# Cobalt-27/CompactFusion

Measured on AMD Instinct MI355X. Metric: residual_compressed_activation_exchange_throughput, higher is better.
Workload: dtype f16

## Files before the change

### compactfusion_amd/csrc/cfx_absmean.hip

```cpp
#include <hip/hip_runtime.h>
#include <hip/hip_ext.h>
#include <stdint.h>
#include <stdio.h>
#include <stdlib.h>
#include <string.h>
#include <algorithm>
#include "cfx.h"
#include "cfx_internal.h"
#include "cfx_device.h"
#include "cfx_host.h"

#define CFX_I_FLAG_LR_FACTORS_ONLY 0x100
#define CFX_I_FLAG_LR_ABS 0x200
extern "C" CFX_HIDDEN size_t cfx_i_lr_workspace_bytes_any(int N, int C, int rank, int batch);
extern "C" CFX_HIDDEN void cfx_i_lr_factor_offsets(int N, int C, int rank, size_t* offU16, size_t* offV16, size_t* per);

template <bool EMIT_BITS, int US, bool WT = false, int NW = WAVES, bool PUB = false, bool KEEP = false, bool TAG = false>
__device__ __forceinline__ void absmean_stats_body(const cfx_comp_item& it, int N, int C, int R, int CB, int bx, int by,
                                                   u64* rowpart, u64 (*sm)[TILE_C], Probe probe = Probe(),
                                                   h16x8* xk = nullptr, h16x8* bk = nullptr, TagArena ta = TagArena()) {
#define SSTAMP(k) probe.at(k)
    const TileCoord t = tile_coord_at(bx, by, N, C, R);
    const int cb = bx;
    u64* colpart = rowpart + (size_t)N * CB;
// ... 263 lines not shown
            for (int k = 0; k < 8; ++k) u[k] = (k0 + k < K) ? U[(size_t)r * K + k0 + k] : (h16)0;
#pragma unroll
            for (int e = 0; e < 8; ++e)
#pragma unroll
                for (int k = 0; k < 8; ++k) acc[j][e] += (float)(h16)(u[k] * v[e][k]);
        }
    }
#pragma unroll
    for (int j = 0; j < RPT; ++j) {
        const int r = t.r0 + t.w + j * WAVES;
        if (r >= t.r1) continue;
        h16x8 bv = (h16x8)(h16)0, xv = (h16x8)(h16)0;
        if (base) bv = ld8(base + (size_t)r * C + t.c);
        unsigned byte;
        if (QUANT) {
            xv = ld8(x + (size_t)r * C + t.c);
            const h16x8 d = xv - bv;
            byte = 0;
#pragma unroll
            for (int i = 0; i < 8; ++i) byte |= (d[i] >= (h16)0 ? 1u : 0u) << i;
            pk[(size_t)r * C8 + (t.c >> 3)] = (unsigned char)byte;
        } else byte = pk[(size_t)r * C8 + (t.c >> 3)];
        if (!upd) continue;
        h16x8 o;
#pragma unroll
        for (int e = 0; e < 8; ++e) {
            const h16 sc = (h16)acc[j][e];
            const h16 recv = ((byte >> e) & 1u) ? sc : -sc;
            o[e] = base ? (h16)(bv[e] + recv) : recv;
        }
        if (QUANT && !ef) o = xv;
        st8(out + (size_t)r * C + t.c, o);
    }
}

#ifndef WATCH_SLEEP
#define WATCH_SLEEP 4
#endif
#ifndef INT2_FLAG_SLEEP
#define INT2_FLAG_SLEEP 2
#endif
__device__ __forceinline__ void scales_watch(const TagArena& ta, int N, int C, int c0, int r0, long long timeout) {
    const int tid = threadIdx.x;
    if (tid < 2) {
        const u64* w = tid ? ta.tU + min(r0, N - 1) : ta.tV + min(c0 + ((r0 >> 1) & (TILE_C - 1)), C - 1);
        SpinClock clk;
        while (!tag_is(ld_wt(w), ta.tagbits)) {
            __builtin_amdgcn_s_sleep(WATCH_SLEEP);
            if (clk.expired(timeout)) break;
        }
    }
    lds_barrier();
}
template <int ROWS, bool WATCH = true>
__device__ __forceinline__ bool scales_from_tagged(const TagArena& ta, int N, int C, int c0, int r0, u16* s16, long long timeout, unsigned* err) {
    static_assert(ROWS <= TILE_C, "one token word per thread (512 threads = the column block's channels)");
    const int tid = threadIdx.x;
    const u64* pv = ta.tV + min(c0 + tid, C - 1);
    const u64* pu = ta.tU + min(r0 + tid, N - 1);
    SpinClock clk;
    if (WATCH) scales_watch(ta, N, C, c0, r0, timeout);
    for (;;) {
        const u64 v = ld_wt(pv);
        const u64 u = tid < ROWS ? ld_wt(pu) : ta.tagbits;
        const bool ok = tag_is(v, ta.tagbits) && tag_is(u, ta.tagbits);
        s16[tid] = (u16)v;
        if (tid < ROWS) s16[TILE_C + tid] = (u16)u;
        if (!__syncthreads_or(ok ? 0 : 1)) return true;
        __builtin_amdgcn_s_sleep(2);
        if (__syncthreads_or(!ok && clk.expired(timeout) ? 1 : 0)) {
            if (tid == 0) gate_fail(err);
            return false;
        }
    }
}

#ifndef ONEBIT_D_TAGGED
#define ONEBIT_D_TAGGED 0
#endif
template <int NW, int KR, int KL, bool ST>
__device__ __forceinline__ void binary_dequant_gated_body(const cfx_decomp_item& it, int N, int C, int R, int tile_x, int tile_y,
                                                         unsigned* gate, unsigned expect, unsigned* err, long long timeout, u32x4* lds,
                                                         Probe probe = Probe(), bool remote = false, bool tagged = false, TagArena ta = TagArena(),
                                                         u16* s16 = nullptr) {
    constexpr int K = KR + KL;
#define GSTAMP(k) do { if (ST && probe.on()) { asm volatile("s_waitcnt vmcnt(0)" ::: "memory"); probe.at(k); } } while (0)
    const TileCoord t = tile_coord_at(tile_x, tile_y, N, C, R);
    if (ST) { probe.at(0); probe.set(7, 4); }
    const unsigned char* pk = (const unsigned char*)it.packet;
    const int C8 = C >> 3;
    const u16* U = (const u16*)(pk + (size_t)N * C8);
    const u16* V = U + N;
    const h16* base = (const h16*)it.base;
    h16* out = (h16*)it.recon;
    const int cc = min(t.c, C - 8);
    h16x8 bv[KR];
    if (base) {
#pragma unroll
        for (int j = 0; j < KR; ++j) bv[j] = ld8nt(base + (size_t)min(t.r0 + t.w + NW * j, t.r1 - 1) * C + cc);
        if constexpr (KL > 0) {
            h16x8 tl[KL > 0 ? KL : 1];
#pragma unroll
            for (int j = 0; j < KL; ++j) tl[j] = ld8nt(base + (size_t)min(t.r0 + t.w + NW * (KR + j), t.r1 - 1) * C + cc);
#pragma unroll
            for (int j = 0; j < KL; ++j) lds[j * (NW * 64) + threadIdx.x] = __builtin_bit_cast(u32x4, tl[j]);
        }
    } else {
#pragma unroll
        for (int j = 0; j < KR; ++j) bv[j] = (h16x8)(h16)0;
    }
    GSTAMP(1);
    h16x8 v8;
    u16 ul;
    unsigned by[K];
    if (tagged) {
        scales_watch(ta, N, C, tile_x * TILE_C, t.r0, timeout);
        if (ST) probe.at(2);
#pragma unroll
        for (int j = 0; j < K; ++j) by[j] = ld_wt(pk + (size_t)min(t.r0 + t.w + NW * j, t.r1 - 1) * C8 + (cc >> 3));
        if (!scales_from_tagged<NW * K, false>(ta, N, C, tile_x * TILE_C, t.r0, s16, timeout, err)) return;
        v8 = __builtin_bit_cast(h16x8, *(const u16x8*)(s16 + 8 * t.lane));
        ul = s16[TILE_C + min(t.w + NW * min(t.lane, K - 1), t.r1 - 1 - t.r0)];
    } else if (!gate_wait<true>(gate, expect, err, timeout)) return;
    else if (remote) {
        if (ST) probe.at(2);
        u16x8 vb;
#pragma unroll
        for (int i = 0; i < 8; ++i) vb[i] = ld_sys(V + cc + i);
        v8 = __builtin_bit_cast(h16x8, vb);
        ul = ld_sys(U + min(t.r0 + t.w + NW * min(t.lane, K - 1), t.r1 - 1));
#pragma unroll
        for (int j = 0; j < K; ++j) by[j] = ld_sys(pk + (size_t)min(t.r0 + t.w + NW * j, t.r1 - 1) * C8 + (cc >> 3));
    } else {
        if (ST) probe.at(2);
        v8 = ld8_wt(V + cc);
        ul = ld_wt(U + min(t.r0 + t.w + NW * min(t.lane, K - 1), t.r1 - 1));
#pragma unroll
        for (int j = 0; j < K; ++j) by[j] = ld_wt(pk + (size_t)min(t.r0 + t.w + NW * j, t.r1 - 1) * C8 + (cc >> 3));
    }
    GSTAMP(3);
#pragma unroll
    for (int j = 0; j < K; ++j) {
        const int rr = t.r0 + t.w + NW * j;
        const h16 uj = hfrom((u16)__builtin_amdgcn_readlane((int)ul, j));
        if (rr < t.r1 && t.act) {
            const h16x8 s = v8 * uj;
            u16x8 sb = __builtin_bit_cast(u16x8, s);
#pragma unroll
            for (int i = 0; i < 8; ++i) sb[i] ^= ((by[j] >> i) & 1u) ? (u16)0 : (u16)0x8000;
            const h16x8 recv = __builtin_bit_cast(h16x8, sb);
            h16x8 bj = (h16x8)(h16)0;
            if (j < KR) bj = bv[j < KR ? j : 0];
            else if (base) bj = __builtin_bit_cast(h16x8, lds[(j - KR) * (NW * 64) + threadIdx.x]);
            st8nt(out + (size_t)rr * C + t.c, base ? (bj + recv) : recv);
        }
    }
    GSTAMP(4);
#undef GSTAMP
}

__device__ __forceinline__ void row_sums2_wt(const u64* rowpart, const unsigned* row32, int N, int CB, int m0, int m1, bool two, u64& s0, u64& s1) {
    s0 = 0; s1 = 0;
    for (int k0 = 0; k0 < CB; k0 += FUSED_RCH) {
        unsigned a[FUSED_RCH], b[FUSED_RCH];
#pragma unroll
        for (int j = 0; j < FUSED_RCH; ++j) a[j] = ld_wt(&row32[(size_t)min(k0 + j, CB - 1) * N + m0]);
        if (two) {
#pragma unroll
            for (int j = 0; j < FUSED_RCH; ++j) b[j] = ld_wt(&row32[(size_t)min(k0 + j, CB - 1) * N + m1]);
        } else {
#pragma unroll
            for (int j = 0; j < FUSED_RCH; ++j) b[j] = 0;
        }
        bool sat = false;
#pragma unroll
        for (int j = 0; j < FUSED_RCH; ++j) {
            s0 += (k0 + j < CB) ? a[j] : 0; s1 += (k0 + j < CB) ? b[j] : 0;
            sat |= (a[j] == PART_SAT) | (b[j] == PART_SAT);
        }
        if (sat) {
            for (int j = 0; j < FUSED_RCH && k0 + j < CB; ++j) {
                if (a[j] == PART_SAT) s0 += ld_wt(&rowpart[(size_t)(k0 + j) * N + m0]) - (u64)PART_SAT;
                if (two && b[j] == PART_SAT) s1 += ld_wt(&rowpart[(size_t)(k0 + j) * N + m1]) - (u64)PART_SAT;
            }
        }
    }
}

template <bool GATED>
__device__ __forceinline__ void absmean_last_arriver_jobs(const cfx_comp_item& it, int N, int C, int CB, int P, int bx, u64* rowpart,
                                                          unsigned* tick, int per_byte, int eps_mode, u64 (*sm)[TILE_C], bool last_col,
                                                          bool last_all, Probe probe, unsigned* gate, unsigned gate_expect) {
    constexpr int NT = FUSED_NT;
#define STAMP(k) probe.at(k)
    lds_barrier();
    const int tid = threadIdx.x;
    const u64* colpart = rowpart + (size_t)N * CB;
    const unsigned* row32 = part32_of(rowpart, N, C, CB);
    const unsigned* col32 = row32 + (size_t)N * CB;
    h16* U = (h16*)((char*)it.packet + (size_t)N * (C / per_byte));
    h16* V = U + N;
    const int c = bx * TILE_C + tid;
// ... 211 lines not shown
    const u16 ul = s16[TILE_C + min(t.w + NW * min(t.lane, US - 1), t.r1 - 1 - t.r0)];
    const bool has_base = it.base != nullptr;
    u16 codes[US];
#pragma unroll
    for (int j = 0; j < US; ++j) {
        const int rr = t.r0 + t.w + NW * j;
        const h16 tk = hfrom((u16)__builtin_amdgcn_readlane((int)ul, j));
        codes[j] = 0;
        if (rr < t.r1 && t.act) {
            const h16x8 d = xk[j] - bk[j];
            const h16x8 thr = ch8 * tk;
            const h16x8 a = habs8(d);
            unsigned code = 0;
#pragma unroll
            for (int i = 0; i < 8; ++i) {
                const unsigned sg = d[i] >= (h16)0 ? 1u : 0u;
                const unsigned m = a[i] > thr[i] ? 1u : 0u;
                code |= ((sg << 1) | m) << (2 * i);
            }
            codes[j] = (u16)code;
            ((u16*)smw)[j * 64 + t.lane] = (u16)code;
        }
    }
    {
        const int j = t.lane >> 3, seg = t.lane & 7;
        const int rr = t.r0 + t.w + NW * j;
        if (t.lane < 8 * US && rr < t.r1 && bx * TILE_C + seg * 64 < C)
            st16_wt(pk + (size_t)rr * (C >> 2) + bx * (TILE_C >> 2) + seg * 16, *(const u32x4*)(smw + j * 128 + seg * 16));
    }
    asm volatile("s_waitcnt vmcnt(0)" ::: "memory");
    lds_barrier();
    if (threadIdx.x == 0) {
        st_wt(&ta.tdone[(size_t)bx * ((N + R - 1) / R) + by], ta.tagbits);
        gate_arrive(gate2, 1u, expect2);
    }
    if (upd) {
#pragma unroll
        for (int j = 0; j < US; ++j) {
            const int rr = t.r0 + t.w + NW * j;
            const h16 tk = hfrom((u16)__builtin_amdgcn_readlane((int)ul, j));
            if (rr < t.r1 && t.act) {
                const h16x8 recv = int2_recv(codes[j], ch8 * tk);
                st8nt(nb + (size_t)rr * C + t.c, ef ? (has_base ? (bk[j] + recv) : recv) : xk[j]);
            }
        }
    }
}

template <bool EMIT_BITS, int US, bool GATED = false, bool KEEP = false>
__device__ __forceinline__ void absmean_fused_body(const cfx_comp_item& it, int N, int C, int R, int CB, int P, int bx, int by,
                                                   u64* rowpart, unsigned* tick, int per_byte, int eps_mode, u64 (*sm)[TILE_C], int dbg,
                                                   Probe probe, unsigned* gate = nullptr, unsigned gate_expect = 0, int flags = 0,
                                                   unsigned* gate2 = nullptr, unsigned expect2 = 0, unsigned* err = nullptr, long long timeout = 0,
                                                   TagArena ta = TagArena()) {
#define STAMP(k) probe.at(k)
    STAMP(0);
#ifdef CFX_DEV_PROBES
    if (dbg == 3) return;
    if (dbg == 4) {
        const TileCoord t = tile_coord_at(bx, by, N, C, R);
        h16x8 acc = (h16x8)(h16)0;
        for (int r = t.r0 + t.w; r < t.r1; r += FUSED_NW * US) {
            h16x8 xv[US], bv[US];
#pragma unroll
            for (int j = 0; j < US; ++j) {
                const int rr = min(r + FUSED_NW * j, t.r1 - 1);
                xv[j] = ld8nt((const h16*)it.x + (size_t)rr * C + min(t.c, C - 8));
                bv[j] = ld8((const h16*)it.base + (size_t)rr * C + min(t.c, C - 8));
            }
#pragma unroll
            for (int j = 0; j < US; ++j) acc += xv[j] - bv[j];
        }
        if (acc[0] == (h16)12345.0f) ((h16*)it.packet)[threadIdx.x] = acc[1];
        return;
    }
#endif
    h16x8 xk[KEEP ? US : 1], bk[KEEP ? US : 1];
    absmean_stats_body<EMIT_BITS, US, true, FUSED_NW, GATED, KEEP, GATED>(it, N, C, R, CB, bx, by, rowpart, sm, probe, xk, bk, ta);
    STAMP(1);
    if constexpr (GATED) {
        const bool v_wg = by == P - 1;
        const bool u_wg = P >= 2 ? (by == P - 2 && bx == CB - 1) : (bx == CB - 1);
        probe.copy(2, 1); probe.copy(3, 1); probe.set(7, (v_wg ? 1 : 0) | (u_wg ? 2 : 0));
        if (v_wg || u_wg) {
            u32x4* park = (u32x4*)&sm[FUSED_NW][0];
            if constexpr (KEEP) {
                park[threadIdx.x] = __builtin_bit_cast(u32x4, xk[US - 1]);
                park[FUSED_NT + threadIdx.x] = __builtin_bit_cast(u32x4, bk[US - 1]);
            }
            absmean_tagged_jobs(it, N, C, CB, P, bx, rowpart, ta, per_byte, eps_mode, sm, v_wg, u_wg, probe, gate, err, timeout);
            if constexpr (KEEP) {
                xk[US - 1] = __builtin_bit_cast(h16x8, park[threadIdx.x]);
                bk[US - 1] = __builtin_bit_cast(h16x8, park[FUSED_NT + threadIdx.x]);
            }
        }
    } else {
    asm volatile("s_waitcnt vmcnt(0)" ::: "memory");
    __syncthreads();
    STAMP(2);
#ifdef CFX_DEV_PROBES
    if (dbg == 1) return;
#endif
    unsigned* flag = (unsigned*)&sm[0][0];
    if (threadIdx.x == 0) flag[0] = __hip_atomic_fetch_add(tick + 1 + bx, 1u, __ATOMIC_RELAXED, __HIP_MEMORY_SCOPE_AGENT);
    if (threadIdx.x == 64) (void)__hip_atomic_fetch_add(tick + TICK_ALL, 1u, __ATOMIC_RELAXED, __HIP_MEMORY_SCOPE_AGENT);
    lds_barrier();
    const bool last_col = flag[0] == (unsigned)(P - 1);
    const bool u_wg = bx == 0 && by == 0;
    STAMP(3);
    probe.set(7, (last_col ? 1 : 0) | (u_wg ? 2 : 0));
#ifdef CFX_DEV_PROBES
    if (dbg == 2) {
        if (last_col && threadIdx.x == 0) st_wt(tick + 1 + bx, 0u);
        if (u_wg && threadIdx.x == 0) {
            while (ld_wt(tick + TICK_ALL) != (unsigned)(CB * P)) __builtin_amdgcn_s_sleep(1);
            st_wt(tick + TICK_ALL, 0u);
        }
        return;
    }
#endif
    if (last_col)
        absmean_last_arriver_jobs<GATED>(it, N, C, CB, P, bx, rowpart, tick, per_byte, eps_mode, sm, true, false, probe, gate, gate_expect);
    if (u_wg) {
        bool failed = false;
        if (threadIdx.x == 0) {
            SpinClock clk;
            while (ld_wt(tick + TICK_ALL) != (unsigned)(CB * P)) {
                __builtin_amdgcn_s_sleep(1);
                if (clk.expired(timeout)) { failed = true; gate_fail(err); break; }
            }
        }
        if (__syncthreads_or(failed ? 1 : 0)) return;
        absmean_last_arriver_jobs<GATED>(it, N, C, CB, P, bx, rowpart, tick, per_byte, eps_mode, sm, false, true, probe, gate, gate_expect);
    }
    }
    if constexpr (KEEP)
        own_tile_finish<US>(it, N, C, R, bx, by, flags, xk, bk, gate, gate_expect, gate2, expect2, err, timeout,
                                       (unsigned char*)&sm[__builtin_amdgcn_readfirstlane(threadIdx.x >> 6)][0], ta, (u16*)&sm[FUSED_NW + 4][0]);
#undef STAMP
}

struct FusedArgs {
    int N, C, CB, R, P;
    int n_st;
    int dq_R, dq_rb;
    int per_byte, eps_mode;
    int dbg;
    u64* ws;
    size_t ws_stride;
    unsigned* tick;
    Probe probe;
    int n_g, g_R, g_rb, n_gt;
    unsigned* gate;
    unsigned gate_expect;
    unsigned* gate_err;
    long long timeout;
    u64* tarena; size_t tarena_stride; unsigned tag;
    signed char src[CFX_MAX_BATCH];
    unsigned* xgate;
    unsigned xexpect;
    int remote;
    P2PInline p2p;
};
#ifndef GATE_WPE
#define GATE_WPE 4
#endif
template <bool EMIT_BITS, int US, bool GATED = false, bool ST = false>
__global__ __launch_bounds__(FUSED_NT, GATE_WPE) __attribute__((amdgpu_num_vgpr(52))) void k_absmean_compress(BatchC batch, BatchD ride, BatchD gated, FusedArgs a) {
    __shared__ u64 sm[FUSED_NW][TILE_C];
    int b = blockIdx.x;
    if (b < a.n_st) {
        const int per = a.CB * a.P;
        const int z = b / per, rem = b - z * per;
        const int by = rem / a.CB;
        absmean_fused_body<EMIT_BITS, US, GATED>(batch.it[z], a.N, a.C, a.R, a.CB, a.P, rem - by * a.CB, by, a.ws + (size_t)z * a.ws_stride,
                                                 a.tick + z * TICK_WORDS, a.per_byte, a.eps_mode, sm, a.dbg,
                                                 a.probe.of(b), a.gate, a.gate_expect, 0, nullptr, 0u, a.gate_err, a.timeout,
                                                 tag_arena_of(a.tarena, a.tarena_stride, z, a.N, a.C, a.CB, a.P, a.tag));
        if constexpr (GATED) {
            if (b == 0 && a.p2p.own) p2p_exchange_inline(a.gate, a.gate_expect, 1, a.p2p, a.xgate, a.xexpect, a.gate_err);
        }
        return;
    }
    if constexpr (EMIT_BITS) {
        b -= a.n_st;
        if constexpr (GATED) {
            if (b < a.n_g) {
                const int per = a.CB * a.g_rb;
                for (int t = b; t < a.n_gt; t += a.n_g) {
                    const int item = t / per, rem = t - item * per;
                    const int ty = rem / a.CB;
                    const int sz = a.src[item];
                    const TagArena ta = tag_arena_of(a.tarena, a.tarena_stride, sz >= 0 ? sz : 0, a.N, a.C, a.CB, a.P, a.tag);
                    binary_dequant_gated_body<FUSED_NW, GATE_KR, 0, ST>(gated.it[item], a.N, a.C, a.g_R, rem - ty * a.CB, ty, a.xgate ? a.xgate : a.gate,
                                                                a.xgate ? a.xexpect : a.gate_expect, a.gate_err, a.timeout,
                                                                nullptr,
                                                                a.probe.of(blockIdx.x), a.remote != 0 && sz < 0,
                                                                ONEBIT_D_TAGGED && sz >= 0, ta, (u16*)&sm[0][0]);
                }
                return;
            }
            b -= a.n_g;
        }
        const int per = a.CB * a.dq_rb;
        const int item = b / per, rem = b - item * per;
        const int ty = rem / a.CB;
        binary_dequant_body<FUSED_NW>(ride.it[item], a.N, a.C, a.dq_R, rem - ty * a.CB, ty);
    }
}

#ifndef PIPE_US
#define PIPE_US 2
#endif
#define PIPE_MAX_DQ CFX_PIPE_MAX_DQ
struct BatchDX { cfx_decomp_item it[PIPE_MAX_DQ]; };
struct PipeArgs {
    int N, C, CB;
    int n_fin, fin_bpi, fin_P;
    int n_st, st_R, st_P;
    int dq_R, dq_rb;
    const u64* ws_fin;
    u64* ws_st;
    size_t ws_stride;
};
template <bool STEADY>
__global__ __launch_bounds__(NTHR) __attribute__((amdgpu_waves_per_eu(8, 8))) void k_binary_pipe(BatchDX dq, BatchC fin, BatchC st, PipeArgs a) {
    __shared__ u64 sm[WAVES][TILE_C];
    int b = blockIdx.x;
    if (b < a.n_fin) {
        const int item = b / a.fin_bpi;
        absmean_finalize_body<NTHR>(fin.it[item], a.N, a.C, a.CB, a.fin_P, 8, 0, a.ws_fin + (size_t)item * a.ws_stride, b - item * a.fin_bpi, &sm[0][0]);
        return;
    }
    b -= a.n_fin;
    if (b < a.n_st) {
        const int per = a.CB * a.st_P;
        const int item = b / per, rem = b - item * per;
        const int ty = rem / a.CB;
        absmean_stats_body<true, PIPE_US>(st.it[item], a.N, a.C, a.st_R, a.CB, rem - ty * a.CB, ty, a.ws_st + (size_t)item * a.ws_stride, sm);
        return;
    }
    b -= a.n_st;
    const int per = a.CB * a.dq_rb;
    const int item = b / per, rem = b - item * per;
    const int ty = rem / a.CB;
    binary_dequant_body<WAVES>(dq.it[item], a.N, a.C, a.dq_R, rem - ty * a.CB, ty);
}


__global__ __launch_bounds__(NTHR) void k_int2_quant(BatchC batch, int N, int C, int R, int flags) {
    const cfx_comp_item it = batch.it[blockIdx.z];
    const TileCoord t = tile_coord(N, C, R);
    const int C4 = C >> 2;
    unsigned char* pk = (unsigned char*)it.packet;
    const h16* TOK = (const h16*)(pk + (size_t)N * C4);
    const h16* CH = TOK + N;
    const h16* x = (const h16*)it.x;
    const h16* base = (const h16*)it.base;
    h16* nb = (h16*)it.new_base;
    const bool upd = (flags & CFX_FLAG_UPDATE_CACHE) && nb;
// ... 312 lines not shown
        a.flags = flags; a.ws = ws; a.ws_stride = wstride; a.tick = tick;
        a.gate1 = ctx->gate + (size_t)slot * GATE_STRIDE;
        a.gate2 = a.gate1 + GATE_BLOCK;
        ctx->gate_expect[3 * slot] += (unsigned)batch * (unsigned)(CB + 1);
        ctx->gate_expect[3 * slot + 1] += (unsigned)a.n_st;
        a.expect1 = ctx->gate_expect[3 * slot]; a.expect2 = ctx->gate_expect[3 * slot + 1];
        a.err = ctx->gate_err;
        a.timeout = ctx->gate_timeout;
        a.tarena_stride = tag_arena_words(N, C, CB, P);
        a.tag = abs_arena_for(ctx, slot / TICK_RING, stream, a.tarena_stride * batch * sizeof(u64), &a.tarena);
        if (!a.tag) return fail(ctx, CFX_ERR_LAUNCH, "2-bit layer launch: cannot allocate the partials' arena");
        for (int g_ = 0; g_ < n_gated; ++g_) {
            a.src[g_] = -1;
            for (int i = 0; i < batch; ++i)
                if (gd.it[g_].packet == items[i].packet) a.src[g_] = (signed char)i;
        }
        if (xg) {
            a.xgate = a.gate1 + 2 * GATE_BLOCK;
            a.xexpect = ++ctx->gate_expect[3 * slot + 2];
            a.remote = xg->remote;
            fill_p2p(ctx, xg, a.p2p);
            xg->taken = 1;
            xg->p_gate = a.gate2 + 1 * GATE_LINE;
            xg->p_expect = a.expect2;
            xg->f_gate = a.xgate; xg->f_expect = a.xexpect;
        }
        const dim3 g(a.n_st + a.n_g);
        LAUNCH(ctx, KID_ABSMEAN_COMPRESS_GATED, s, (k_int2_compress_gated<4>), g, dim3(FUSED_NT), 0, s, b, gd, a);
        return check_launch(ctx, "2-bit layer launch");
    }
    const bool ef_gated = one_launch && codec == CFX_CODEC_BINARY && upd && !(flags & CFX_FLAG_NO_EF) && n_gated + batch <= CFX_MAX_BATCH;
    const bool one_launch_1bit = one_launch && codec == CFX_CODEC_BINARY && (!upd || ef_gated);
    int n_gated_k = n_gated;
    if (ef_gated) {
        for (int i = n_gated - 1; i >= 0; --i) gd.it[i + batch] = gd.it[i];
        for (int i = 0; i < batch; ++i) { gd.it[i].packet = items[i].packet; gd.it[i].base = items[i].base; gd.it[i].recon = items[i].new_base; }
        n_gated_k = n_gated + batch;
    }
    if (fused) {
        FusedArgs a;
        memset(&a, 0, sizeof(a));
        a.N = N; a.C = C; a.CB = CB; a.R = R; a.P = P;
        a.n_st = CB * P * batch;
        a.dq_R = FUSED_NW * UNROLL;
        a.dq_rb = (N + a.dq_R - 1) / a.dq_R;
        a.per_byte = per_byte; a.eps_mode = codec == CFX_CODEC_INT2 ? 1 : 0;
        a.ws = ws; a.ws_stride = wstride; a.tick = tick;
        a.dbg = ctx->dev_probe;
        a.probe = cfx_i_probe(ctx);
        if (one_launch_1bit) {
            a.g_rb = (N + FUSED_NW * GATE_KR - 1) / (FUSED_NW * GATE_KR);
            a.g_R = ((N + a.g_rb - 1) / a.g_rb + FUSED_NW - 1) / FUSED_NW * FUSED_NW;
            a.n_gt = a.n_g = CB * a.g_rb * n_gated_k;
            a.gate = ctx->gate + (size_t)slot * GATE_STRIDE;
            ctx->gate_expect[3 * slot] += (unsigned)batch * (unsigned)(CB + 1);
            a.gate_expect = ctx->gate_expect[3 * slot];
            a.tarena_stride = tag_arena_words(N, C, CB, P);
            a.tag = abs_arena_for(ctx, slot / TICK_RING, stream, a.tarena_stride * batch * sizeof(u64), &a.tarena);
            if (!a.tag) return fail(ctx, CFX_ERR_LAUNCH, "1-bit layer launch: cannot allocate the partials' arena");
            for (int g_ = 0; g_ < n_gated_k; ++g_) {
                a.src[g_] = -1;
                for (int i = 0; i < batch; ++i)
                    if (gd.it[g_].packet == items[i].packet) a.src[g_] = (signed char)i;
            }
            if (xg) {
                a.xgate = a.gate + GATE_BLOCK;
                a.xexpect = ++ctx->gate_expect[3 * slot + 1];
                a.remote = xg->remote;
                fill_p2p(ctx, xg, a.p2p);
                xg->taken = 1;
                xg->p_gate = a.gate; xg->p_expect = a.gate_expect;
                xg->f_gate = a.xgate; xg->f_expect = a.xexpect;
            }
        }
        a.gate_err = ctx->gate_err;
        a.timeout = ctx->gate_timeout;
        const dim3 g(a.n_st + a.n_g + CB * a.dq_rb * n_ride);
#ifdef CFX_DEV_PROBES
        if (one_launch_1bit && ctx->dev_buf && R % 32 == 0) {
            LAUNCH(ctx, KID_ABSMEAN_COMPRESS_GATED, s, (k_absmean_compress<true, 4, true, true>), g, dim3(FUSED_NT), 0, s, b, rd, gd, a);
        } else
#endif
        if (one_launch_1bit) {
            LAUNCH(ctx, KID_ABSMEAN_COMPRESS_GATED, s, (k_absmean_compress<true, 4, true>), g, dim3(FUSED_NT), 0, s, b, rd, gd, a);
        } else if (codec == CFX_CODEC_BINARY) {
            if (R % 32 == 0) LAUNCH(ctx, KID_ABSMEAN_COMPRESS_BITS, s, (k_absmean_compress<true, 4>), g, dim3(FUSED_NT), 0, s, b, rd, gd, a);
            else LAUNCH(ctx, KID_ABSMEAN_COMPRESS_BITS, s, (k_absmean_compress<true, 2>), g, dim3(FUSED_NT), 0, s, b, rd, gd, a);
        } else {
            if (R % 32 == 0) LAUNCH(ctx, KID_ABSMEAN_COMPRESS, s, (k_absmean_compress<false, 4>), g, dim3(FUSED_NT), 0, s, b, rd, gd, a);
            else LAUNCH(ctx, KID_ABSMEAN_COMPRESS, s, (k_absmean_compress<false, 2>), g, dim3(FUSED_NT), 0, s, b, rd, gd, a);
        }
    } else {
        if (codec == CFX_CODEC_BINARY) LAUNCH(ctx, KID_ABSMEAN_STATS_BITS, s, k_absmean_stats<true>, grid, dim3(NTHR), 0, s, b, N, C, R, ws, wstride);
        else LAUNCH(ctx, KID_ABSMEAN_STATS, s, k_absmean_stats<false>, grid, dim3(NTHR), 0, s, b, N, C, R, ws, wstride);
        LAUNCH(ctx, KID_ABSMEAN_FINALIZE, s, k_absmean_finalize, dim3(1 + (C + 255) / 256, batch), dim3(1024), 0, s, b, N, C, CB, P, per_byte,
                           codec == CFX_CODEC_INT2 ? 1 : 0, (const u64*)ws, wstride);
        if (n_ride) {
            const int Rr = auto_rows(ctx, N, C, n_ride, false);
            LAUNCH(ctx, KID_BINARY_DEQUANT, s, k_binary_dequant<UNROLL>, dim3(CB, (N + Rr - 1) / Rr, n_ride), dim3(NTHR), 0, s, rd, N, C, Rr, (unsigned*)nullptr, 0u);
        }
    }
    if (codec == CFX_CODEC_INT2) {
        LAUNCH(ctx, KID_INT2_QUANT, s, k_int2_quant, gridq, dim3(NTHR), 0, s, b, N, C, Rq, flags);
    } else if (upd && !one_launch_1bit) {
        if (flags & CFX_FLAG_NO_EF) {
            for (int i = 0; i < batch; ++i)
                if (items[i].new_base != items[i].x)
                    hipLaunchKernelGGL(k_copy_probe, dim3(2048), dim3(256), 0, s, (uint4*)items[i].new_base, (const uint4*)items[i].x, (size_t)N * C * 2 / 16);
        } else {
            BatchD d;
            memset(&d, 0, sizeof(d));
            for (int i = 0; i < batch; ++i) { d.it[i].packet = items[i].packet; d.it[i].base = items[i].base; d.it[i].recon = items[i].new_base; }
            LAUNCH(ctx, KID_BINARY_EF, s, k_binary_dequant<UNROLL>, gridq, dim3(NTHR), 0, s, d, N, C, Rq, (unsigned*)nullptr, 0u);
        }
    }
    if (n_gated && !(one_launch_1bit || (one_launch && codec == CFX_CODEC_INT2))) {
        const int Rg = auto_rows(ctx, N, C, n_gated, false);
        if (codec == CFX_CODEC_BINARY) LAUNCH(ctx, KID_BINARY_DEQUANT, s, k_binary_dequant<UNROLL>, dim3(CB, (N + Rg - 1) / Rg, n_gated), dim3(NTHR), 0, s, gd, N, C, Rg, (unsigned*)nullptr, 0u);
        else LAUNCH(ctx, KID_INT2_DEQUANT, s, k_int2_dequant, dim3(CB, (N + Rg - 1) / Rg, n_gated), dim3(NTHR), 0, s, gd, N, C, Rg, (unsigned*)nullptr, 0u);
    }
    return check_launch(ctx, "compress launch");
}

int cfx_i_absmean_decompress(cfx_ctx* ctx, int codec, int N, int C, int batch, const BatchD& b, int R, void* stream, unsigned* pre, unsigned pre_val) {
    hipStream_t s = (hipStream_t)stream;
    const dim3 grid((C + TILE_C - 1) / TILE_C, (N + R - 1) / R, batch);
    if (codec == CFX_CODEC_BINARY) {
        if (stream_cu_count(ctx, stream) < 128) {
            const int R4 = WAVES * 4;
            LAUNCH(ctx, KID_BINARY_DEQUANT, s, k_binary_dequant<4>, dim3(grid.x, (N + R4 - 1) / R4, batch), dim3(NTHR), 0, s, b, N, C, R4, pre, pre_val);
// ... 153 lines not shown
```

### compactfusion_amd/csrc/cfx_api.hip

```cpp
#include <hip/hip_runtime.h>
#include <hip/hip_ext.h>
#include <stdint.h>
#include <stdio.h>
#include <stdlib.h>
#include <string.h>
#include <algorithm>
#include "cfx.h"
#include "cfx_internal.h"
#include "cfx_device.h"
#define CFX_API_TU
#include "cfx_host.h"

__global__ __launch_bounds__(256) void k_residual2_delta(const h16* __restrict__ x, const h16* base, const h16* dbase, h16* dd, size_t n8) {
    const size_t i = (size_t)blockIdx.x * 256 + threadIdx.x;
    if (i >= n8) return;
    const h16x8 d = ld8nt(x + i * 8) - ld8(base + i * 8);
    st8(dd + i * 8, d - ld8(dbase + i * 8));
}
__global__ __launch_bounds__(256) void k_residual2_update(const h16* base, const h16* dbase, const h16* __restrict__ recv, h16* nb, h16* ndb,
                                                          float decay, size_t n8) {
    const size_t i = (size_t)blockIdx.x * 256 + threadIdx.x;
    if (i >= n8) return;
    const h16x8 b = ld8(base + i * 8), d = ld8(dbase + i * 8), r = ld8nt(recv + i * 8);
    const h16x8 pred = b + d;
// ... 111 lines not shown
    c->err[0] = 0;
    return c;
}

int cfx_prepare(cfx_ctx* ctx) {
    if (!ctx) return CFX_ERR_NULL;
    if (ctx->tick) return CFX_OK;
    int cur = -1;
    (void)hipGetDevice(&cur);
    if (cur != ctx->device && hipSetDevice(ctx->device) != hipSuccess) return fail(ctx, CFX_ERR_LAUNCH, "prepare: hipSetDevice failed");
    static_assert(3 * TICK_RING * CFX_RING_STREAMS == sizeof(((cfx_ctx*)0)->gate_expect) / sizeof(unsigned), "gate_expect has three entries per ring slot");
    const size_t tick_words = (size_t)CFX_RING_STREAMS * TICK_RING * CFX_MAX_BATCH * TICK_WORDS;
    const size_t gate_words = (size_t)(CFX_RING_STREAMS * TICK_RING + 1) * GATE_STRIDE;
    const size_t colgate_words = (size_t)CFX_RING_STREAMS * MML_MAX_TILES;
    const size_t bytes = (tick_words + gate_words + colgate_words) * sizeof(unsigned);
    void* p = nullptr;
    int rc = CFX_OK;
    if (hipMalloc(&p, bytes) != hipSuccess || hipMemset(p, 0, bytes) != hipSuccess || hipDeviceSynchronize() != hipSuccess) {
        (void)hipGetLastError();
        if (p) (void)hipFree(p);
        rc = fail(ctx, CFX_ERR_LAUNCH, "prepare: cannot allocate the ticket blocks");
    } else {
        ctx->tick = (unsigned*)p;
        ctx->gate = ctx->tick + tick_words;
        ctx->colgate = ctx->gate + gate_words;
        ctx->mml_seq = 0;
        void* e = nullptr;
        if (hipHostMalloc(&e, 64, hipHostMallocMapped) != hipSuccess) { (void)hipGetLastError(); (void)hipFree(p); ctx->tick = nullptr; rc = fail(ctx, CFX_ERR_LAUNCH, "prepare: cannot allocate the error word"); }
        else { memset(e, 0, 64); ctx->gate_err = (unsigned*)e; }
        memset(ctx->gate_expect, 0, sizeof(ctx->gate_expect));
    }
    if (cur >= 0 && cur != ctx->device) (void)hipSetDevice(cur);
    return rc;
}

#ifdef CFX_DEV_PROBES
int cfx_dev_stamps(cfx_ctx* ctx, void* buf) {
    if (!ctx) return CFX_ERR_NULL;
    ctx->dev_buf = buf;
    return CFX_OK;
}

int cfx_dev_set_launch_tags(cfx_ctx* ctx, unsigned abs_seq, unsigned mml_seq) {
    if (!ctx) return CFX_ERR_NULL;
    if (!ctx->tick && cfx_prepare(ctx) != CFX_OK) return CFX_ERR_LAUNCH;
    (void)hipDeviceSynchronize();
    ctx->abs_seq = abs_seq;
    ctx->mml_seq = mml_seq;
    return CFX_OK;
}

int cfx_dev_set_probe(cfx_ctx* ctx, int mode) {
    if (!ctx) return CFX_ERR_NULL;
    if (mode < 0 || mode > 4) return fail(ctx, CFX_ERR_BATCH, "dev probe must be 0..4");
    ctx->dev_probe = mode;
    return CFX_OK;
}
#endif

int cfx_set_fused_finalize(cfx_ctx* ctx, int on) {
    if (!ctx) return CFX_ERR_NULL;
    ctx->fused = on != 0;
    return CFX_OK;
}

int cfx_set_stats_rows(cfx_ctx* ctx, int rows) {
    if (!ctx) return CFX_ERR_NULL;
    if (rows < 0 || rows > 4096) return fail(ctx, CFX_ERR_BATCH, "stats rows must be 0 (automatic) .. 4096");
    ctx->stats_rows = rows;
    return CFX_OK;
}

int cfx_set_gated_launch(cfx_ctx* ctx, int on) {
    if (!ctx) return CFX_ERR_NULL;
    ctx->gated_on = on != 0;
    return CFX_OK;
}

int cfx_set_lr_chain(cfx_ctx* ctx, int chain) {
    if (!ctx) return CFX_ERR_NULL;
    if (chain < 0 || chain > 2) return fail(ctx, CFX_ERR_BATCH, "lr chain must be 0 (automatic), 1 (no single launch) or 2 (C-space chain)");
    ctx->lr_chain = chain;
    return CFX_OK;
}

int cfx_set_lr_decode(cfx_ctx* ctx, int mode) {
    if (!ctx) return CFX_ERR_NULL;
    if (mode < 0 || mode > 2) return fail(ctx, CFX_ERR_BATCH, "lr decode must be 0 (automatic), 1 (VALU) or 2 (MFMA)");
    ctx->lr_decode = mode;
    return CFX_OK;
}

int cfx_set_allow_shared_queues(cfx_ctx* ctx, int on) {
    if (!ctx) return CFX_ERR_NULL;
    ctx->allow_shared_queues = on != 0;
    return CFX_OK;
}

int cfx_hw_queues_ok(void) {
    static int ok = -1;
    if (ok < 0) {
        const char* v = getenv("GPU_MAX_HW_QUEUES");
        ok = (v && atoi(v) >= 2) ? 1 : 0;
    }
    return ok;
}

// ... 388 lines not shown
```

### compactfusion_amd/csrc/cfx_device.h

```cpp
#ifndef CFX_DEVICE_H
#define CFX_DEVICE_H
#include <hip/hip_runtime.h>
#include <stdint.h>
#include "cfx.h"
#include "cfx_internal.h"

typedef _Float16 h16;
typedef h16 h16x8 __attribute__((ext_vector_type(8)));
typedef unsigned short u16;
typedef u16 u16x8 __attribute__((ext_vector_type(8)));
typedef unsigned long long u64;

#define TILE_C 512
#define WAVES 4
#define NTHR (WAVES * 64)
#define UNROLL 2
#define UNROLL_S 4

struct BatchC { cfx_comp_item it[CFX_MAX_BATCH]; };
struct BatchD { cfx_decomp_item it[CFX_MAX_BATCH]; };

__device__ __forceinline__ u16 hbits(h16 v) { return __builtin_bit_cast(u16, v); }
__device__ __forceinline__ h16 hfrom(u16 v) { return __builtin_bit_cast(h16, v); }

// ... 123 lines not shown
        const h16 lvl = (idx & 1u) ? (h16)2.0 * thr[i] : (h16)0.5 * thr[i];
        r[i] = (idx & 2u) ? lvl : -lvl;
    }
    return r;
}

struct TileCoord {
    int lane, w, c, r0, r1;
    bool act;
};
__device__ __forceinline__ TileCoord tile_coord_at(int bx, int by, int N, int C, int R) {
    TileCoord t;
    t.lane = threadIdx.x & 63;
    t.w = __builtin_amdgcn_readfirstlane(threadIdx.x >> 6);
    t.c = bx * TILE_C + t.lane * 8;
    t.act = t.c < C;
    t.r0 = by * R;
    t.r1 = min(N, t.r0 + R);
    return t;
}
__device__ __forceinline__ TileCoord tile_coord(int N, int C, int R) { return tile_coord_at(blockIdx.x, blockIdx.y, N, C, R); }

#define MML_MAX_TILES 2048
#define TICK_WORDS 64
#define TICK_ALL 48
#define TICK_MAX_CB 46
#define TICK_RING 256

#define FUSED_NW 8
#define FUSED_NT (FUSED_NW * 64)
#ifndef FUSED_CH
#define FUSED_CH 18

#endif
#define FUSED_RCH 6

#ifndef GATE_KR
#define GATE_KR 14
#endif
#ifndef GATE_KR2
#define GATE_KR2 17

#endif
#ifndef GATE_KL
#define GATE_KL 6
#endif
#define GATE_LDS_ROWS ((GATE_KL * FUSED_NT * 16 + TILE_C * 8 - 1) / (TILE_C * 8))
#ifndef GATE_LOCAL_SLEEP
#define GATE_LOCAL_SLEEP 1

#endif
#define GATE_LINE 16
#define GATE_BLOCK (25 * GATE_LINE)
#define GATE_STRIDE (3 * GATE_BLOCK)
__device__ __forceinline__ void gate_arrive_few(unsigned* gate, unsigned inc) {
    (void)__hip_atomic_fetch_add(gate, inc, __ATOMIC_RELAXED, __HIP_MEMORY_SCOPE_AGENT);
}
__device__ __forceinline__ void gate_arrive(unsigned* gate, unsigned inc, unsigned expect) {
    const unsigned old = __hip_atomic_fetch_add(gate, inc, __ATOMIC_RELAXED, __HIP_MEMORY_SCOPE_AGENT);
    if (old + inc == expect) {
#pragma unroll
        for (int x = 0; x < 8; ++x) st_wt(gate + (1 + x) * GATE_LINE, expect);
    }
}
__device__ __forceinline__ unsigned ld_l2(const unsigned* p) {
    unsigned v;
    asm volatile("global_load_dword %0, %1, off nt\n\ts_waitcnt vmcnt(0)" : "=&v"(v) : "v"(p) : "memory");
    return v;
}
struct SpinClock {
    long long t0 = 0;
    __device__ __forceinline__ bool expired(long long timeout) {
        const long long now = wall_clock64();
        if (!t0) { t0 = now; return false; }
        return now - t0 > timeout;
    }
};
template <bool FEW = false>
__device__ __forceinline__ bool gate_wait(unsigned* gate, unsigned expect, unsigned* err, long long timeout) {
    bool failed = false;
    if (threadIdx.x == 0) {
        const unsigned xcc = __builtin_amdgcn_s_getreg((3 << 11) | 20) & 7u;
        unsigned* open = FEW ? gate : gate + (1 + xcc) * GATE_LINE;
        unsigned* local = gate + (9 + xcc) * GATE_LINE;
        unsigned* claim = gate + (17 + xcc) * GATE_LINE;
        const bool relay = __hip_atomic_exchange(claim, expect, __ATOMIC_RELAXED, __HIP_MEMORY_SCOPE_AGENT) != expect;
        SpinClock clk;
        unsigned n = 0;
        if (relay) {
            while (ld_wt(open) != expect) {
                __builtin_amdgcn_s_sleep(1);
                if (clk.expired(timeout)) { failed = true; break; }
            }
            if (!failed) *(volatile unsigned*)local = expect;
        } else {
            while (ld_l2(local) != expect) {
                if (GATE_LOCAL_SLEEP) __builtin_amdgcn_s_sleep(GATE_LOCAL_SLEEP);
                ++n;
                if ((n & (FEW ? 255u : 15u)) == 0) {
                    if (ld_wt(open) == expect) break;
                    if (clk.expired(timeout)) { failed = true; break; }
                }
            }
        }
        if (failed) gate_fail(err);
    }
    return __syncthreads_or(failed ? 1 : 0) == 0;
}
__device__ __forceinline__ h16x8 ld8_wt(const u16* p) {
    if ((((uintptr_t)p) & 7) == 0) {
        struct { u64 a, b; } q = {ld_wt((const u64*)p), ld_wt((const u64*)p + 1)};
        return __builtin_bit_cast(h16x8, q);
    }
    u16x8 vb;
#pragma unroll
    for (int i = 0; i < 8; ++i) vb[i] = ld_wt(p + i);
    return __builtin_bit_cast(h16x8, vb);
}

struct P2PInline {
    unsigned* own;
    const unsigned* peer[CFX_P2P_MAX_PEERS];
    int n_peers;
    long long timeout;
};
__device__ __forceinline__ unsigned ld_sys32(const unsigned* p) { return __hip_atomic_load(p, __ATOMIC_RELAXED, __HIP_MEMORY_SCOPE_SYSTEM); }
__device__ __forceinline__ void p2p_exchange_inline(const unsigned* p_gate, unsigned p_expect, int p_count, const P2PInline& p,
                                                    unsigned* f_gate, unsigned f_expect, unsigned* err) {
    if ((threadIdx.x >> 6) != 0) return;
    const int lane = threadIdx.x & 63;
    const long long t0 = wall_clock64();
    unsigned epoch = 0;
    if (lane == 0) epoch = ld_sys32(p.own) + 1u;
    bool gave_up = false;
    for (;;) {
        bool behind = false;
        for (int i = lane; i < p_count; i += 64) behind |= (int)(ld_wt(p_gate + i) - p_expect) < 0;
        if (__builtin_amdgcn_ballot_w64(behind) == 0) break;
        __builtin_amdgcn_s_sleep(1);
        if (wall_clock64() - t0 > p.timeout) { gave_up = true; break; }
    }
    if (__builtin_amdgcn_ballot_w64(gave_up) != 0) { if (lane == 0) gate_fail(err); return; }
    if (lane == 0) __hip_atomic_store(p.own, epoch, __ATOMIC_RELAXED, __HIP_MEMORY_SCOPE_SYSTEM);
    epoch = (unsigned)__builtin_amdgcn_readfirstlane((int)epoch);
    if (lane < p.n_peers) {
        while ((int)(ld_sys32(p.peer[lane]) - epoch) < 0) {
            __builtin_amdgcn_s_sleep(2);
            if (wall_clock64() - t0 > p.timeout) { gave_up = true; break; }
        }
    }
    if (__builtin_amdgcn_ballot_w64(gave_up) != 0) { if (lane == 0) gate_fail(err); return; }
    if (lane == 0) st_wt(f_gate, f_expect);
}


static __global__ __launch_bounds__(256) void k_copy_probe(uint4* __restrict__ dst, const uint4* __restrict__ src, size_t n16) {
    typedef unsigned u32x4_ __attribute__((ext_vector_type(4)));
    const u32x4_* s4 = reinterpret_cast<const u32x4_*>(src);
    u32x4_* d4 = reinterpret_cast<u32x4_*>(dst);
    const size_t per = (n16 + gridDim.x - 1) / gridDim.x;
    const size_t b0 = (size_t)blockIdx.x * per, b1 = b0 + per < n16 ? b0 + per : n16;
// ... 13 lines not shown
```

Before: 2087.

## Add chained tagged-stats workgroups with per-XCC relay gates and packed bit loads

Adds dedicated chain workgroups at the front of the gated fused kernel. They compute the tagged abs-mean stats jobs, then one workgroup per XCC claims a relay role and publishes a per-XCC tag-open flag or gate copy. Gated dequant workgroups spin on this local per-XCC line instead of polling the scattered tag words. The dequant also loads sign bits as 32-bit words covering four rows and redistributes them with ds_bpermute, which cuts the number of byte loads. This adds more grid blocks, head sleeps and relay spin loops, so synchronization latency and scheduling could get worse.

Result: no change. 2094, median of 6 (+0.3%).

```diff
diff --git a/compactfusion_amd/csrc/cfx_absmean.hip b/compactfusion_amd/csrc/cfx_absmean.hip
--- a/compactfusion_amd/csrc/cfx_absmean.hip
+++ b/compactfusion_amd/csrc/cfx_absmean.hip
@@ -339,6 +339,22 @@
     }
     lds_barrier();
 }
+__device__ __forceinline__ void scales_open_wait(const unsigned* open, unsigned tag, const TagArena& ta, int N, int C, int c0, int r0, long long timeout) {
+    if (threadIdx.x == 0) {
+        const u64* wv = ta.tV + min(c0 + ((r0 >> 1) & (TILE_C - 1)), C - 1);
+        const u64* wu = ta.tU + min(r0, N - 1);
+        SpinClock clk;
+        unsigned n = 0;
+        while (ld_l2(open) != tag) {
+            if (GATE_LOCAL_SLEEP) __builtin_amdgcn_s_sleep(GATE_LOCAL_SLEEP);
+            if ((++n & 255u) == 0) {
+                if (tag_is(ld_wt(wv), ta.tagbits) && tag_is(ld_wt(wu), ta.tagbits)) break;
+                if (clk.expired(timeout)) break;
+            }
+        }
+    }
+    lds_barrier();
+}
 template <int ROWS, bool WATCH = true>
 __device__ __forceinline__ bool scales_from_tagged(const TagArena& ta, int N, int C, int c0, int r0, u16* s16, long long timeout, unsigned* err) {
     static_assert(ROWS <= TILE_C, "one token word per thread (512 threads = the column block's channels)");
@@ -365,11 +381,27 @@
 #ifndef ONEBIT_D_TAGGED
 #define ONEBIT_D_TAGGED 0
 #endif
+template <int K, int NW, bool SYS>
+__device__ __forceinline__ void bits4_load(unsigned (&by4)[(K + 3) / 4], const unsigned char* pk, const TileCoord& t, int tile_x, int C8) {
+    const int off = min(tile_x * (TILE_C >> 3) + (t.lane & 15) * 4, C8 - 4);
+#pragma unroll
+    for (int i = 0; i < (K + 3) / 4; ++i) {
+        const int j = min((t.lane >> 4) + 4 * i, K - 1);
+        const unsigned* p = (const unsigned*)(pk + (size_t)min(t.r0 + t.w + NW * j, t.r1 - 1) * C8 + off);
+        by4[i] = SYS ? ld_sys32(p) : ld_wt(p);
+    }
+}
+template <int K>
+__device__ __forceinline__ unsigned bits4_byte(const unsigned (&by4)[(K + 3) / 4], int j, int lane) {
+    const unsigned w = (unsigned)__builtin_amdgcn_ds_bpermute((((j & 3) << 4) | (lane >> 2)) << 2, (int)by4[j >> 2]);
+    return (w >> ((lane & 3) * 8)) & 0xffu;
+}
+
 template <int NW, int KR, int KL, bool ST>
 __device__ __forceinline__ void binary_dequant_gated_body(const cfx_decomp_item& it, int N, int C, int R, int tile_x, int tile_y,
                                                          unsigned* gate, unsigned expect, unsigned* err, long long timeout, u32x4* lds,
                                                          Probe probe = Probe(), bool remote = false, bool tagged = false, TagArena ta = TagArena(),
-                                                         u16* s16 = nullptr) {
+                                                         u16* s16 = nullptr, const unsigned* tagopen = nullptr, bool defer = false) {
     constexpr int K = KR + KL;
 #define GSTAMP(k) do { if (ST && probe.on()) { asm volatile("s_waitcnt vmcnt(0)" ::: "memory"); probe.at(k); } } while (0)
     const TileCoord t = tile_coord_at(tile_x, tile_y, N, C, R);
@@ -381,6 +413,10 @@
     const h16* base = (const h16*)it.base;
     h16* out = (h16*)it.recon;
     const int cc = min(t.c, C - 8);
+    if (defer) {
+        if (tagged) scales_open_wait(tagopen, (unsigned)(ta.tagbits >> 40), ta, N, C, tile_x * TILE_C, t.r0, timeout);
+        else if (!gate_wait<true>(gate, expect, err, timeout)) return;
+    }
     h16x8 bv[KR];
     if (base) {
 #pragma unroll
@@ -399,16 +435,17 @@
     GSTAMP(1);
     h16x8 v8;
     u16 ul;
-    unsigned by[K];
+    unsigned by4[(K + 3) / 4];
     if (tagged) {
-        scales_watch(ta, N, C, tile_x * TILE_C, t.r0, timeout);
+        if (defer) {}
+        else if (tagopen) scales_open_wait(tagopen, (unsigned)(ta.tagbits >> 40), ta, N, C, tile_x * TILE_C, t.r0, timeout);
+        else scales_watch(ta, N, C, tile_x * TILE_C, t.r0, timeout);
         if (ST) probe.at(2);
-#pragma unroll
-        for (int j = 0; j < K; ++j) by[j] = ld_wt(pk + (size_t)min(t.r0 + t.w + NW * j, t.r1 - 1) * C8 + (cc >> 3));
+        bits4_load<K, NW, false>(by4, pk, t, tile_x, C8);
         if (!scales_from_tagged<NW * K, false>(ta, N, C, tile_x * TILE_C, t.r0, s16, timeout, err)) return;
         v8 = __builtin_bit_cast(h16x8, *(const u16x8*)(s16 + 8 * t.lane));
         ul = s16[TILE_C + min(t.w + NW * min(t.lane, K - 1), t.r1 - 1 - t.r0)];
-    } else if (!gate_wait<true>(gate, expect, err, timeout)) return;
+    } else if (!defer && !gate_wait<true>(gate, expect, err, timeout)) return;
     else if (remote) {
         if (ST) probe.at(2);
         u16x8 vb;
@@ -416,25 +453,24 @@
         for (int i = 0; i < 8; ++i) vb[i] = ld_sys(V + cc + i);
         v8 = __builtin_bit_cast(h16x8, vb);
         ul = ld_sys(U + min(t.r0 + t.w + NW * min(t.lane, K - 1), t.r1 - 1));
-#pragma unroll
-        for (int j = 0; j < K; ++j) by[j] = ld_sys(pk + (size_t)min(t.r0 + t.w + NW * j, t.r1 - 1) * C8 + (cc >> 3));
+        bits4_load<K, NW, true>(by4, pk, t, tile_x, C8);
     } else {
         if (ST) probe.at(2);
         v8 = ld8_wt(V + cc);
         ul = ld_wt(U + min(t.r0 + t.w + NW * min(t.lane, K - 1), t.r1 - 1));
-#pragma unroll
-        for (int j = 0; j < K; ++j) by[j] = ld_wt(pk + (size_t)min(t.r0 + t.w + NW * j, t.r1 - 1) * C8 + (cc >> 3));
+        bits4_load<K, NW, false>(by4, pk, t, tile_x, C8);
     }
     GSTAMP(3);
 #pragma unroll
     for (int j = 0; j < K; ++j) {
         const int rr = t.r0 + t.w + NW * j;
         const h16 uj = hfrom((u16)__builtin_amdgcn_readlane((int)ul, j));
+        const unsigned byj = bits4_byte<K>(by4, j, t.lane);
         if (rr < t.r1 && t.act) {
             const h16x8 s = v8 * uj;
             u16x8 sb = __builtin_bit_cast(u16x8, s);
 #pragma unroll
-            for (int i = 0; i < 8; ++i) sb[i] ^= ((by[j] >> i) & 1u) ? (u16)0 : (u16)0x8000;
+            for (int i = 0; i < 8; ++i) sb[i] ^= ((byj >> i) & 1u) ? (u16)0 : (u16)0x8000;
             const h16x8 recv = __builtin_bit_cast(h16x8, sb);
             h16x8 bj = (h16x8)(h16)0;
             if (j < KR) bj = bv[j < KR ? j : 0];
@@ -752,7 +788,7 @@
                                                    u64* rowpart, unsigned* tick, int per_byte, int eps_mode, u64 (*sm)[TILE_C], int dbg,
                                                    Probe probe, unsigned* gate = nullptr, unsigned gate_expect = 0, int flags = 0,
                                                    unsigned* gate2 = nullptr, unsigned expect2 = 0, unsigned* err = nullptr, long long timeout = 0,
-                                                   TagArena ta = TagArena()) {
+                                                   TagArena ta = TagArena(), bool chain = false) {
 #define STAMP(k) probe.at(k)
     STAMP(0);
 #ifdef CFX_DEV_PROBES
@@ -779,8 +815,8 @@
     absmean_stats_body<EMIT_BITS, US, true, FUSED_NW, GATED, KEEP, GATED>(it, N, C, R, CB, bx, by, rowpart, sm, probe, xk, bk, ta);
     STAMP(1);
     if constexpr (GATED) {
-        const bool v_wg = by == P - 1;
-        const bool u_wg = P >= 2 ? (by == P - 2 && bx == CB - 1) : (bx == CB - 1);
+        const bool v_wg = !chain && by == P - 1;
+        const bool u_wg = !chain && (P >= 2 ? (by == P - 2 && bx == CB - 1) : (bx == CB - 1));
         probe.copy(2, 1); probe.copy(3, 1); probe.set(7, (v_wg ? 1 : 0) | (u_wg ? 2 : 0));
         if (v_wg || u_wg) {
             u32x4* park = (u32x4*)&sm[FUSED_NW][0];
@@ -843,6 +879,7 @@
 struct FusedArgs {
     int N, C, CB, R, P;
     int n_st;
+    int n_chain, n_jobs, relay_tag, relay_gate;
     int dq_R, dq_rb;
     int per_byte, eps_mode;
     int dbg;
@@ -865,10 +902,22 @@
 #ifndef GATE_WPE
 #define GATE_WPE 4
 #endif
+#ifndef CHAIN_TAGGED
+#define CHAIN_TAGGED 1
+#endif
+#ifndef CHAIN_HEAD_SLEEP
+#define CHAIN_HEAD_SLEEP 6
+#endif
+__device__ __forceinline__ void absmean_chain_workgroup(const BatchC& batch, const FusedArgs& a, int c, u64 (*sm)[TILE_C]);
+
 template <bool EMIT_BITS, int US, bool GATED = false, bool ST = false>
 __global__ __launch_bounds__(FUSED_NT, GATE_WPE) __attribute__((amdgpu_num_vgpr(52))) void k_absmean_compress(BatchC batch, BatchD ride, BatchD gated, FusedArgs a) {
     __shared__ u64 sm[FUSED_NW][TILE_C];
     int b = blockIdx.x;
+    if constexpr (GATED) {
+        if (b < a.n_chain) { absmean_chain_workgroup(batch, a, b, sm); return; }
+        b -= a.n_chain;
+    }
     if (b < a.n_st) {
         const int per = a.CB * a.P;
         const int z = b / per, rem = b - z * per;
@@ -876,9 +925,9 @@
         absmean_fused_body<EMIT_BITS, US, GATED>(batch.it[z], a.N, a.C, a.R, a.CB, a.P, rem - by * a.CB, by, a.ws + (size_t)z * a.ws_stride,
                                                  a.tick + z * TICK_WORDS, a.per_byte, a.eps_mode, sm, a.dbg,
                                                  a.probe.of(b), a.gate, a.gate_expect, 0, nullptr, 0u, a.gate_err, a.timeout,
-                                                 tag_arena_of(a.tarena, a.tarena_stride, z, a.N, a.C, a.CB, a.P, a.tag));
+                                                 tag_arena_of(a.tarena, a.tarena_stride, z, a.N, a.C, a.CB, a.P, a.tag), GATED && a.n_chain > 0);
         if constexpr (GATED) {
-            if (b == 0 && a.p2p.own) p2p_exchange_inline(a.gate, a.gate_expect, 1, a.p2p, a.xgate, a.xexpect, a.gate_err);
+            if (b == 0 && a.n_chain == 0 && a.p2p.own) p2p_exchange_inline(a.gate, a.gate_expect, 1, a.p2p, a.xgate, a.xexpect, a.gate_err);
         }
         return;
     }
@@ -887,6 +936,14 @@
         if constexpr (GATED) {
             if (b < a.n_g) {
                 const int per = a.CB * a.g_rb;
+                unsigned xcc = __builtin_amdgcn_s_getreg((3 << 11) | 20) & 7u;
+                bool defer = false;
+#ifdef CFX_DEV_PROBES
+                if (a.dbg == 7) xcc = (xcc + 1u) & 7u;
+                defer = a.dbg == 5;
+                if (ST) a.probe.of(blockIdx.x).set(8, cu_where());
+#endif
+                const unsigned* tagopen = a.gate + GATE_TAGOPEN + xcc * GATE_LINE;
                 for (int t = b; t < a.n_gt; t += a.n_g) {
                     const int item = t / per, rem = t - item * per;
                     const int ty = rem / a.CB;
@@ -896,7 +953,8 @@
                                                                 a.xgate ? a.xexpect : a.gate_expect, a.gate_err, a.timeout,
                                                                 nullptr,
                                                                 a.probe.of(blockIdx.x), a.remote != 0 && sz < 0,
-                                                                ONEBIT_D_TAGGED && sz >= 0, ta, (u16*)&sm[0][0]);
+                                                                sz >= 0 && (ONEBIT_D_TAGGED || a.relay_tag), ta, (u16*)&sm[0][0],
+                                                                a.relay_tag ? tagopen : nullptr, defer);
                 }
                 return;
             }
@@ -906,6 +964,55 @@
         const int item = b / per, rem = b - item * per;
         const int ty = rem / a.CB;
         binary_dequant_body<FUSED_NW>(ride.it[item], a.N, a.C, a.dq_R, rem - ty * a.CB, ty);
+    }
+}
+
+__device__ __forceinline__ void absmean_chain_workgroup(const BatchC& batch, const FusedArgs& a, int c, u64 (*sm)[TILE_C]) {
+    const Probe probe = a.probe.of((size_t)a.n_st + c);
+    probe.at(0); probe.set(7, 8);
+    unsigned* const rgate = a.xgate ? a.xgate : a.gate;
+    const unsigned rexpect = a.xgate ? a.xexpect : a.gate_expect;
+    unsigned xcc = __builtin_amdgcn_s_getreg((3 << 11) | 20) & 7u;
+    bool want = a.relay_tag || a.relay_gate;
+#ifdef CFX_DEV_PROBES
+    probe.set(8, cu_where());
+    if (a.dbg == 6) want = false;
+    if (a.dbg == 7) xcc = (xcc + 2u) & 7u;
+#endif
+    bool relay = false;
+    if (want && threadIdx.x < 64) {
+        if (threadIdx.x == 0) relay = gate_relay_claim(rgate, rexpect, xcc);
+        relay = __builtin_amdgcn_readfirstlane(relay ? 1 : 0) != 0;
+    }
+    for (int i = 0; i < CHAIN_HEAD_SLEEP; ++i) __builtin_amdgcn_s_sleep(16);
+    for (int j = c; j < a.n_jobs; j += a.n_chain) {
+        const int z = j / (a.CB + 1), k = j - z * (a.CB + 1);
+        absmean_tagged_jobs(batch.it[z], a.N, a.C, a.CB, a.P, min(k, a.CB - 1), a.ws + (size_t)z * a.ws_stride,
+                            tag_arena_of(a.tarena, a.tarena_stride, z, a.N, a.C, a.CB, a.P, a.tag), a.per_byte, a.eps_mode, sm, k < a.CB, k == a.CB,
+                            probe, a.gate, a.gate_err, a.timeout);
+    }
+    if (relay && a.relay_tag) {
+        const int lane = threadIdx.x;
+        SpinClock clk;
+        bool gave_up = false;
+        for (;;) {
+            bool behind = false;
+            for (int j = lane; j < a.n_jobs; j += 64) {
+                const int z = j / (a.CB + 1), k = j - z * (a.CB + 1);
+                const TagArena ta = tag_arena_of(a.tarena, a.tarena_stride, z, a.N, a.C, a.CB, a.P, a.tag);
+                behind |= !tag_is(ld_wt(k < a.CB ? ta.tV + min(k * TILE_C + TILE_C - 1, a.C - 1) : ta.tU + (a.N - 1)), ta.tagbits);
+            }
+            if (__builtin_amdgcn_ballot_w64(behind) == 0) break;
+            __builtin_amdgcn_s_sleep(1);
+            if (clk.expired(a.timeout)) { gave_up = true; break; }
+        }
+        if (lane == 0 && !gave_up) *(volatile unsigned*)(a.gate + GATE_TAGOPEN + xcc * GATE_LINE) = a.tag;
+        probe.at(10);
+    }
+    if (c == 0 && a.p2p.own) p2p_exchange_inline(a.gate, a.gate_expect, 1, a.p2p, a.xgate, a.xexpect, a.gate_err);
+    if (relay && a.relay_gate && threadIdx.x == 0) {
+        gate_relay_run(rgate, rexpect, xcc, a.gate_err, a.timeout);
+        probe.at(9);
     }
 }
 
@@ -1324,17 +1431,23 @@
             a.g_rb = (N + FUSED_NW * GATE_KR - 1) / (FUSED_NW * GATE_KR);
             a.g_R = ((N + a.g_rb - 1) / a.g_rb + FUSED_NW - 1) / FUSED_NW * FUSED_NW;
             a.n_gt = a.n_g = CB * a.g_rb * n_gated_k;
+            a.n_jobs = batch * (CB + 1);
+            a.n_chain = std::min(std::max(16, (a.n_jobs + 7) / 8 * 8), 64);
             a.gate = ctx->gate + (size_t)slot * GATE_STRIDE;
             ctx->gate_expect[3 * slot] += (unsigned)batch * (unsigned)(CB + 1);
             a.gate_expect = ctx->gate_expect[3 * slot];
             a.tarena_stride = tag_arena_words(N, C, CB, P);
             a.tag = abs_arena_for(ctx, slot / TICK_RING, stream, a.tarena_stride * batch * sizeof(u64), &a.tarena);
             if (!a.tag) return fail(ctx, CFX_ERR_LAUNCH, "1-bit layer launch: cannot allocate the partials' arena");
+            int n_own = 0;
             for (int g_ = 0; g_ < n_gated_k; ++g_) {
                 a.src[g_] = -1;
                 for (int i = 0; i < batch; ++i)
                     if (gd.it[g_].packet == items[i].packet) a.src[g_] = (signed char)i;
-            }
+                n_own += a.src[g_] >= 0;
+            }
+            a.relay_tag = CHAIN_TAGGED && !xg && n_own > 0;
+            a.relay_gate = xg ? !xg->needs_room : n_own < n_gated_k;
             if (xg) {
                 a.xgate = a.gate + GATE_BLOCK;
                 a.xexpect = ++ctx->gate_expect[3 * slot + 1];
@@ -1347,7 +1460,7 @@
         }
         a.gate_err = ctx->gate_err;
         a.timeout = ctx->gate_timeout;
-        const dim3 g(a.n_st + a.n_g + CB * a.dq_rb * n_ride);
+        const dim3 g(a.n_chain + a.n_st + a.n_g + CB * a.dq_rb * n_ride);
 #ifdef CFX_DEV_PROBES
         if (one_launch_1bit && ctx->dev_buf && R % 32 == 0) {
             LAUNCH(ctx, KID_ABSMEAN_COMPRESS_GATED, s, (k_absmean_compress<true, 4, true, true>), g, dim3(FUSED_NT), 0, s, b, rd, gd, a);
diff --git a/compactfusion_amd/csrc/cfx_api.hip b/compactfusion_amd/csrc/cfx_api.hip
--- a/compactfusion_amd/csrc/cfx_api.hip
+++ b/compactfusion_amd/csrc/cfx_api.hip
@@ -187,7 +187,7 @@
 
 int cfx_dev_set_probe(cfx_ctx* ctx, int mode) {
     if (!ctx) return CFX_ERR_NULL;
-    if (mode < 0 || mode > 4) return fail(ctx, CFX_ERR_BATCH, "dev probe must be 0..4");
+    if (mode < 0 || mode > 7) return fail(ctx, CFX_ERR_BATCH, "dev probe must be 0..7");
     ctx->dev_probe = mode;
     return CFX_OK;
 }
diff --git a/compactfusion_amd/csrc/cfx_device.h b/compactfusion_amd/csrc/cfx_device.h
--- a/compactfusion_amd/csrc/cfx_device.h
+++ b/compactfusion_amd/csrc/cfx_device.h
@@ -199,7 +199,8 @@
 #endif
 #define GATE_LINE 16
 #define GATE_BLOCK (25 * GATE_LINE)
-#define GATE_STRIDE (3 * GATE_BLOCK)
+#define GATE_TAGOPEN (3 * GATE_BLOCK)
+#define GATE_STRIDE (3 * GATE_BLOCK + 8 * GATE_LINE)
 __device__ __forceinline__ void gate_arrive_few(unsigned* gate, unsigned inc) {
     (void)__hip_atomic_fetch_add(gate, inc, __ATOMIC_RELAXED, __HIP_MEMORY_SCOPE_AGENT);
 }
@@ -254,6 +255,24 @@
     }
     return __syncthreads_or(failed ? 1 : 0) == 0;
 }
+__device__ __forceinline__ bool gate_relay_claim(unsigned* gate, unsigned expect, unsigned xcc) {
+    return __hip_atomic_exchange(gate + (17 + xcc) * GATE_LINE, expect, __ATOMIC_RELAXED, __HIP_MEMORY_SCOPE_AGENT) != expect;
+}
+__device__ __forceinline__ void gate_relay_run(unsigned* gate, unsigned expect, unsigned xcc, unsigned* err, long long timeout) {
+    SpinClock clk;
+    while (ld_wt(gate) != expect) {
+        __builtin_amdgcn_s_sleep(1);
+        if (clk.expired(timeout)) { gate_fail(err); return; }
+    }
+    *(volatile unsigned*)(gate + (9 + xcc) * GATE_LINE) = expect;
+}
+
+__device__ __forceinline__ unsigned cu_where() {
+    const unsigned hw = __builtin_amdgcn_s_getreg((32 - 1) << 11 | 4);
+    const unsigned xcc = __builtin_amdgcn_s_getreg((3 << 11) | 20) & 7u;
+    const unsigned key = ((hw >> 8) & 0x1fu) | (((hw >> 13) & 3u) << 5);
+    return (xcc << 8) | key;
+}
 __device__ __forceinline__ h16x8 ld8_wt(const u16* p) {
     if ((((uintptr_t)p) & 7) == 0) {
         struct { u64 a, b; } q = {ld_wt((const u64*)p), ld_wt((const u64*)p + 1)};
```
